# soedinglab/metaeuk

Hardware: AMD Instinct MI355X
Metric: prefilter+align ORF-fragments/sec (hits UNVERIFIED in this run: no CPU reference digest) (higher is better)
Workload: dtype packed i16 / i32 DP on u8 residues, i8 scores

## Files before the change

metaeuk_amd/csrc/mk_sw.hip:

```cpp
#include "mk_kernels.hpp"
#include <algorithm>
#include <mutex>

namespace mk {

template <int G>
__device__ __forceinline__ uint32_t shift_up(uint32_t top, uint32_t x, int laneInGroup) {
    if constexpr (G == 16) {
        return (uint32_t) __builtin_amdgcn_update_dpp((int) top, (int) x, 0x111 , 0xf, 0xf, false);
    } else if constexpr (G == 64) {
        return (uint32_t) __builtin_amdgcn_update_dpp((int) top, (int) x, 0x138 , 0xf, 0xf, false);
    } else {
        const uint32_t v = (uint32_t) __builtin_amdgcn_update_dpp((int) top, (int) x, 0x138 , 0xf, 0xf, false);
        return laneInGroup == 0 ? top : v;
    }
}

template <int G>
__device__ __forceinline__ uint32_t shift_up_zero(uint32_t x, int laneInGroup) {
    if constexpr (G == 16) return (uint32_t) __builtin_amdgcn_update_dpp((int) x, (int) x, 0x111 , 0xf, 0xf, true);
    else return shift_up<G>(0u, x, laneInGroup);
}

__device__ __forceinline__ int max3i(int a, int b, int c) { return max(max(a, b), c); }

template <int R>
__device__ __forceinline__ void load_scores(const int8_t *p, int (&sc)[R]) {
    if constexpr (R == 2) {
        const uint32_t w = *reinterpret_cast<const uint16_t *>(p);
        sc[0] = (int) (int8_t) (w & 0xFF);
        sc[1] = (int) (int8_t) (w >> 8);
    } else {
        const uint32_t *pw = reinterpret_cast<const uint32_t *>(p);
#pragma unroll
        for (int k = 0; k < R / 4; k++) {
            const uint32_t w = pw[k];
            sc[4 * k + 0] = (int) (int8_t) (w & 0xFF);
            sc[4 * k + 1] = (int) (int8_t) ((w >> 8) & 0xFF);
            sc[4 * k + 2] = (int) (int8_t) ((w >> 16) & 0xFF);
            sc[4 * k + 3] = (int) (int8_t) (w >> 24);
        }
    }
}

template <int G, int R, int BLOCK, bool SHARED>
__device__ __forceinline__ void sw_unit(const SwLaunch &L, const uint32_t unit, int8_t *smem, const int8_t *sMat) {
    constexpr int GPB = BLOCK / G;
    constexpr int ROWS = G * R;
    static_assert(!SHARED || BLOCK == 64, "shared-query mode runs one wave per workgroup");
    const int lane = threadIdx.x % G;
    const int grp = threadIdx.x / G;
    uint64_t jobId;
    bool have;
    SwJob job;
    uint32_t profQStart = 0; int profQStep = 1;
    if constexpr (SHARED) {
        const uint32_t w0 = L.wave_start[unit], w1 = L.wave_start[unit + 1];
        const uint32_t count = min((uint32_t) GPB, w1 - w0);
        have = (uint32_t) grp < count;
        jobId = (uint64_t) w0 + (have ? grp : 0);
        job = L.jobs[L.order ? (uint64_t) L.order[jobId] : jobId];
        if (!have) job.t_len = 0;
    } else {
        jobId = (uint64_t) unit * GPB + grp;
        have = jobId < L.n_jobs;
        if (have) job = L.jobs[L.order ? (uint64_t) L.order[jobId] : jobId];
        else { job.t_start = 0; job.q_start = 0; job.q_len = 0; job.t_len = 0; job.q_step = 1; job.t_step = 1; job.slot = 0; }
    }
    profQStart = job.q_start; profQStep = job.q_step;
    int8_t *prof = SHARED ? smem : smem + (size_t) grp * 24 * ROWS;
    const int go = L.gap_open, ge = L.gap_extend;
    const int qLen = (int) job.q_len, tLen = (int) job.t_len;
    const int nTiles = (qLen + ROWS - 1) / ROWS;
    uint32_t *border = L.boundary ? L.boundary + (jobId - L.boundary_job0) * (uint64_t) L.boundary_stride : nullptr;

    constexpr int NEED = (G - 1 + 15) / 16;
    int known = -1, after = 0;
    if constexpr (!SHARED) { if (L.known_score && have && nTiles == 1) known = L.known_score[job.slot]; }
    uint32_t bestKey = 0;
    int bestRow = 0;
    for (int tile = 0; tile < nTiles; tile++) {
        const int row0 = tile * ROWS;
        if (L.q_prof) {
            for (int i = SHARED ? (int) threadIdx.x : lane; i < ROWS * 6; i += SHARED ? BLOCK : G) {
                const int row = i / 6, w = i - row * 6;
                const int q = row0 + row;
                uint32_t v = 0;
                if (q < qLen) v = *reinterpret_cast<const uint32_t *>(L.q_prof + ((int64_t) profQStart + (int64_t) q * profQStep) * 32 + w * 4);
#pragma unroll
                for (int k = 0; k < 4; k++) if (4 * w + k < 22) prof[(4 * w + k) * ROWS + row] = (int8_t) (v >> (8 * k));
            }
        } else {
            uint8_t *sQ = reinterpret_cast<uint8_t *>(prof) + 22 * ROWS;
            int8_t *sB = reinterpret_cast<int8_t *>(sQ) + ROWS;
            for (int row = SHARED ? (int) threadIdx.x : lane; row < ROWS; row += SHARED ? BLOCK : G) {
                const int q = row0 + row;
                const bool real = q < qLen;
                const int64_t qi = (int64_t) profQStart + (int64_t) (real ? q : 0) * profQStep;
                sQ[row] = real ? L.q_res[qi] : (uint8_t) 255;
                sB[row] = real ? L.q_bias8[qi] : (int8_t) 0;
            }
            __builtin_amdgcn_fence(__ATOMIC_ACQ_REL, "wavefront");
            __builtin_amdgcn_wave_barrier();
            for (int idx = SHARED ? (int) threadIdx.x : lane; idx < 22 * ROWS; idx += SHARED ? BLOCK : G) {
                const int t = idx / ROWS, row = idx - t * ROWS;
                const uint32_t qc = sQ[row];
                prof[idx] = (t < 21 && qc != 255u) ? (int8_t) ((int) sMat[t * 21 + (int) qc] + (int) sB[row]) : (int8_t) 0;
            }
        }
        __builtin_amdgcn_fence(__ATOMIC_ACQ_REL, "wavefront");
        __builtin_amdgcn_wave_barrier();

        int H[R], E[R];
        uint32_t key[R];
#pragma unroll
        for (int r = 0; r < R; r++) { H[r] = 0; E[r] = 0; key[r] = 0; }
        uint32_t out0 = 0, out1 = 21u;
        int hupPrev = 0;
        const int steps = tLen > 0 ? tLen + G - 1 : 0;
        const bool readTop = (tile > 0);
        const bool writeBottom = (tile + 1 < nTiles);
        const int laneRow = (int) (threadIdx.x & 15u);
        const int64_t tBase = (int64_t) job.t_start;
        const int64_t tStep = (int64_t) job.t_step;
        const int tLast = max(tLen - 1, 0);
        uint32_t tq0 = L.t_res[tBase + (int64_t) min(laneRow, tLast) * tStep], tq1 = L.t_res[tBase + (int64_t) min(16 + laneRow, tLast) * tStep],
                 tq2 = L.t_res[tBase + (int64_t) min(32 + laneRow, tLast) * tStep];
        for (int s0 = 0; s0 < steps; s0 += 16) {
            uint32_t tcur = tq0;
            tq0 = tq1; tq1 = tq2;
            tq2 = L.t_res[tBase + (int64_t) min(s0 + 48 + laneRow, tLast) * tStep];
            const int sEnd = min(s0 + 16, steps);
            for (int s = s0; s < sEnd; s++) {
                uint32_t top0 = 0;
                const uint32_t top1 = s < tLen ? tcur : 21u;
                tcur = (uint32_t) __builtin_amdgcn_update_dpp(0, (int) tcur, 0x12F , 0xf, 0xf, false);
                if (readTop && lane == 0 && s < tLen) top0 = border[s];
                const uint32_t in0 = shift_up<G>(top0, out0, lane);
                const uint32_t tres = shift_up<G>(top1, out1, lane);
                const int hup = (int) (in0 & 0xFFFFu);
                int F = (int) (in0 >> 16);
                const int c = s - lane;
                const uint32_t cinv = 0x1FFFFu - (uint32_t) max(c, 0);
                int sc[R];
                load_scores<R>(prof + tres * ROWS + lane * R, sc);
                int dsave = hupPrev;
#pragma unroll
                for (int r = 0; r < R; r++) {
                    const int d = min(dsave + sc[r], 32767);
                    dsave = H[r];
                    const int h = max3i(d, E[r], F);
                    key[r] = max(key[r], ((uint32_t) h << 17) | cinv);
                    const int ho = h - go;
                    E[r] = max3i(E[r] - ge, ho, 0);
                    F = max3i(F - ge, ho, 0);
                    H[r] = h;
                }
                hupPrev = hup;
                out0 = (uint32_t) H[R - 1] | ((uint32_t) F << 16);
                out1 = tres;
                if (writeBottom && lane == G - 1 && c >= 0 && c < tLen) border[c] = out0;
            }
            if constexpr (!SHARED) {
                if (known > 0) {
                    bool seen = false;
#pragma unroll
                    for (int r = 0; r < R; r++) seen |= (key[r] >> 17) == (uint32_t) known;
                    const unsigned long long m = __ballot(seen);
                    const unsigned long long mine = G == 64 ? ~0ull : ((1ull << (G & 63)) - 1ull) << (((unsigned) threadIdx.x & 63u) / G * G);
                    if ((m & mine) != 0ull && ++after > NEED) break;
                }
            }
        }
#pragma unroll
        for (int r = 0; r < R; r++) {
            if (key[r] > bestKey) { bestKey = key[r]; bestRow = row0 + lane * R + r; }
        }
        __builtin_amdgcn_fence(__ATOMIC_ACQ_REL, "wavefront");
        __builtin_amdgcn_wave_barrier();
    }
#pragma unroll
    for (int m = G / 2; m >= 1; m >>= 1) {
        const uint32_t ok = (uint32_t) __shfl_xor((int) bestKey, m, G);
        const int orow = __shfl_xor(bestRow, m, G);
        if (ok > bestKey || (ok == bestKey && orow < bestRow)) { bestKey = ok; bestRow = orow; }
    }
    if (have && lane == 0) {
        SwOut o;
        o.score = (int32_t) (bestKey >> 17);
        o.end_col = o.score > 0 ? (int32_t) (0x1FFFFu - (bestKey & 0x1FFFFu)) : -1;
        o.end_row = o.score > 0 ? bestRow : -1;
        o.pad = 0;
        L.out[job.slot] = o;
    }
}

#ifndef MK_HELPER_PRIO
#define MK_HELPER_PRIO 3
#endif
template <int G, int R, int BLOCK, bool SHARED>
__global__ __launch_bounds__(BLOCK) void sw_kernel(SwLaunch L) {
    if (!SHARED && MK_HELPER_PRIO) __builtin_amdgcn_s_setprio(MK_HELPER_PRIO);
    extern __shared__ __attribute__((aligned(16))) int8_t smem[];
    __shared__ int8_t sMat[448];
    for (int k = (int) threadIdx.x; k < 441; k += BLOCK) sMat[k] = L.mat[k];
    __syncthreads();
    if constexpr (SHARED) {
        for (uint32_t done = 0; L.units_per_block == 0 || done < L.units_per_block; done++) {
            uint32_t u = 0;
            if (threadIdx.x == 0) u = atomicAdd(L.work_counter, 1u);
            u = (uint32_t) __builtin_amdgcn_readfirstlane((int) u);
            if ((uint64_t) u >= L.n_waves) break;
            sw_unit<G, R, BLOCK, true>(L, u, smem, sMat);
            __builtin_amdgcn_fence(__ATOMIC_ACQ_REL, "wavefront");
            __builtin_amdgcn_wave_barrier();
        }
    } else {
        sw_unit<G, R, BLOCK, false>(L, blockIdx.x, smem, sMat);
    }
}

template <int CLS>
__global__ __launch_bounds__(64) void sw_multi_kernel(SwLaunch L, const uint32_t *bounds, uint32_t *counter, int prio) {
    if (prio) __builtin_amdgcn_s_setprio(MK_HELPER_PRIO);
    extern __shared__ __attribute__((aligned(16))) int8_t smem[];
    __shared__ int8_t sMat[448];
    for (int k = (int) threadIdx.x; k < 441; k += 64) sMat[k] = L.mat[k];
    __builtin_amdgcn_fence(__ATOMIC_ACQ_REL, "wavefront");
    __builtin_amdgcn_wave_barrier();
    constexpr int C0 = CLS == 0 ? 0 : (CLS == 1 ? 3 : 7), C1 = CLS == 0 ? 3 : (CLS == 1 ? 7 : SW_NCFG), NC = C1 - C0;
    uint32_t lo[NC], nj[NC], ub[NC + 1];
    ub[0] = 0;
#pragma unroll
    for (int k = 0; k < NC; k++) {
        const int c = C1 - 1 - k;
        lo[k] = bounds[c]; nj[k] = bounds[c + 1] - lo[k];
        const uint32_t gpb = c >= 9 ? 1u : (c >= 7 ? 2u : 4u);
        ub[k + 1] = ub[k] + (nj[k] + gpb - 1u) / gpb;
    }
    for (;;) {
        uint32_t u = 0;
        if (threadIdx.x == 0) u = atomicAdd(counter, 1u);
        u = (uint32_t) __builtin_amdgcn_readfirstlane((int) u);
        if (u >= ub[NC]) break;
        int k = 0;
#pragma unroll
        for (int j = 1; j < NC; j++) if (u >= ub[j]) k = j;
        SwLaunch Lc = L;
        uint32_t first = 0, base = 0, count = 0;
#pragma unroll
        for (int j = 0; j < NC; j++) if (j == k) { first = lo[j]; base = ub[j]; count = nj[j]; }
        Lc.order = L.order + first; Lc.n_jobs = count;
        const uint32_t unit = u - base;
        const int c = C1 - 1 - k;
        if constexpr (CLS == 0) {
            if (c == 0) sw_unit<16, 2, 64, false>(Lc, unit, smem, sMat);
            else sw_unit<16, 4, 64, false>(Lc, unit, smem, sMat);
        } else if constexpr (CLS == 1) {
            if (c <= 4) sw_unit<16, 8, 64, false>(Lc, unit, smem, sMat);
            else sw_unit<16, 16, 64, false>(Lc, unit, smem, sMat);
        } else {
            if (c == 7) sw_unit<32, 12, 64, false>(Lc, unit, smem, sMat);
            else if (c == 8) sw_unit<32, 16, 64, false>(Lc, unit, smem, sMat);
            else if (c == 9) sw_unit<64, 12, 64, false>(Lc, unit, smem, sMat);
            else sw_unit<64, 16, 64, false>(Lc, unit, smem, sMat);
        }
        __builtin_amdgcn_fence(__ATOMIC_ACQ_REL, "wavefront");
        __builtin_amdgcn_wave_barrier();
    }
}

hipError_t launch_sw_multi(const SwLaunch &L, const uint32_t *bounds, uint32_t *counter, int cls, uint32_t blocks, hipStream_t stream, bool prio) {
    if (!L.order || !bounds || !counter || L.boundary || blocks == 0) return hipErrorInvalidValue;
    switch (cls) {
        case 0: hipLaunchKernelGGL((sw_multi_kernel<0>), dim3(blocks), dim3(64), (size_t) 64 * 24 * 4, stream, L, bounds, counter, prio ? 1 : 0); break;
        case 1: hipLaunchKernelGGL((sw_multi_kernel<1>), dim3(blocks), dim3(64), (size_t) 64 * 24 * 16, stream, L, bounds, counter, prio ? 1 : 0); break;
        case 2: hipLaunchKernelGGL((sw_multi_kernel<2>), dim3(blocks), dim3(64), (size_t) 64 * 24 * 16, stream, L, bounds, counter, prio ? 1 : 0); break;
        default: return hipErrorInvalidValue;
    }
    return hipGetLastError();
}

typedef short pk16 __attribute__((ext_vector_type(2)));
__device__ __forceinline__ pk16 pk_from(uint32_t v) { return __builtin_bit_cast(pk16, v); }
__device__ __forceinline__ uint32_t pk_bits(pk16 v) { return __builtin_bit_cast(uint32_t, v); }
__device__ __forceinline__ pk16 pk_max(pk16 a, pk16 b) { return __builtin_elementwise_max(a, b); }
__device__ __forceinline__ pk16 pk_splat(int v) { pk16 r; r.x = (short) v; r.y = (short) v; return r; }
typedef unsigned short pku16 __attribute__((ext_vector_type(2)));
__device__ __forceinline__ pk16 pk_subs0(pk16 a, pk16 b) {
    return __builtin_bit_cast(pk16, __builtin_elementwise_sub_sat(__builtin_bit_cast(pku16, a), __builtin_bit_cast(pku16, b)));
}

constexpr uint32_t SWT_MAX_ROWS = 256;
constexpr int SWT_MARGIN = 16, SWT_TAIL = 32, SWT_COL = 24;
__host__ __device__ inline size_t swt_image_bytes(int qLen) { return (size_t) (SWT_MARGIN + qLen + SWT_TAIL) * SWT_COL; }

template <int R>
__device__ __forceinline__ void swt_unit(const SwLaunch &L, const uint32_t w0, const uint32_t count, const int qLen) {
    constexpr int G = 16;
    constexpr int UNR = R <= 2 ? 16 : (R <= 4 ? 8 : (R <= 8 ? 4 : 2));
    extern __shared__ __attribute__((aligned(16))) int8_t smem[];
    const int lane = threadIdx.x % G, grp = threadIdx.x / G;
    const pk16 go2 = pk_splat(L.gap_open), ge2 = pk_splat(L.gap_extend), zero2 = pk_splat(0);
    const bool haveA = (uint32_t) (2 * grp) < count, haveB = (uint32_t) (2 * grp + 1) < count;
    const SwJob jobA = L.jobs[L.order[(uint64_t) w0 + (haveA ? 2 * grp : 0)]];
    const SwJob jobB = L.jobs[L.order[(uint64_t) w0 + (haveB ? 2 * grp + 1 : 0)]];
    const int tLenA = haveA ? (int) jobA.t_len : 0, tLenB = haveB ? (int) jobB.t_len : 0;
    uint32_t offA[R], offB[R];
#pragma unroll
    for (int r = 0; r < R; r++) {
        const int i = lane * R + r;
        const uint32_t a = i < tLenA ? (uint32_t) L.t_res[(int64_t) jobA.t_start + (int64_t) i * jobA.t_step] : 21u;
        const uint32_t b = i < tLenB ? (uint32_t) L.t_res[(int64_t) jobB.t_start + (int64_t) i * jobB.t_step] : 21u;
        offA[r] = min(a, 21u) + (uint32_t) ((SWT_MARGIN - lane) * SWT_COL); offB[r] = min(b, 21u) + (uint32_t) ((SWT_MARGIN - lane) * SWT_COL);
    }
    pk16 H[R], E[R], best[R];
#pragma unroll
    for (int r = 0; r < R; r++) { H[r] = zero2; E[r] = zero2; best[r] = zero2; }
    pk16 hupPrev = zero2;
    uint32_t outH = 0, outF = 0;
    const int steps = (qLen + G - 1 + 15) & ~15;
#pragma unroll 1
    for (int s0 = 0; s0 < steps; s0 += UNR) {
#pragma unroll
        for (int k = 0; k < UNR; k++) {
            const pk16 hup = pk_from(shift_up_zero<G>(outH, lane));
            pk16 F = pk_from(shift_up_zero<G>(outF, lane));
            pk16 dsave = hupPrev;
#pragma unroll
            for (int r = 0; r < R; r++) {
                const int sa = (int) smem[offA[r] + (uint32_t) (k * SWT_COL)], sb = (int) smem[offB[r] + (uint32_t) (k * SWT_COL)];
                const pk16 sc = pk_from(__builtin_amdgcn_perm((uint32_t) sb, (uint32_t) sa, 0x05040100u));
                const pk16 d = dsave + sc;
                dsave = H[r];
                const pk16 h = pk_max(pk_max(d, E[r]), F);
                best[r] = pk_max(best[r], h);
                const pk16 ho = pk_subs0(h, go2);
                E[r] = pk_max(pk_subs0(E[r], ge2), ho);
                F = pk_max(pk_subs0(F, ge2), ho);
                H[r] = h;
            }
            hupPrev = hup;
            outH = pk_bits(H[R - 1]);
            outF = pk_bits(F);
        }
#pragma unroll
        for (int r = 0; r < R; r++) { offA[r] += (uint32_t) (UNR * SWT_COL); offB[r] += (uint32_t) (UNR * SWT_COL); }
    }
    pk16 bAll = zero2;
#pragma unroll
    for (int r = 0; r < R; r++) bAll = pk_max(bAll, best[r]);
    uint32_t b = pk_bits(bAll);
#pragma unroll
    for (int m = G / 2; m >= 1; m >>= 1) b = pk_bits(pk_max(pk_from(b), pk_from((uint32_t) __shfl_xor((int) b, m, G))));
    uint32_t cA = 0x7FFFFFFFu, cB = 0x7FFFFFFFu;
#pragma unroll
    for (int r = R - 1; r >= 0; r--) {
        if ((pk_bits(best[r]) & 0xFFFFu) == (b & 0xFFFFu)) cA = (uint32_t) (lane * R + r);
        if ((pk_bits(best[r]) >> 16) == (b >> 16)) cB = (uint32_t) (lane * R + r);
    }
// ... 146 lines not shown
                for (int s = 0; s < 8; s++) {
                    if (run) {
                        const int k = __ffs((int) run) - 1;
                        run &= run - 1u;
                        jobIdx[s] = (uint32_t) __shfl((int) myJob, k, 64);
                        n++;
                    } else jobIdx[s] = jobIdx[0];
                }
                if constexpr (CLS == 0) {
                    if (tl <= 32u) swtp_unit<2>(L, jobIdx, n, (int) qLen);
                    else if (tl <= 48u) swtp_unit<3>(L, jobIdx, n, (int) qLen);
                    else swtp_unit<4>(L, jobIdx, n, (int) qLen);
                } else if constexpr (CLS == 1) {
                    if (tl <= 96u) swtp_unit<6>(L, jobIdx, n, (int) qLen);
                    else swtp_unit<8>(L, jobIdx, n, (int) qLen);
                } else {
                    if (tl <= 192u) swtp_unit<12>(L, jobIdx, n, (int) qLen);
                    else swtp_unit<16>(L, jobIdx, n, (int) qLen);
                }
            }
            __builtin_amdgcn_fence(__ATOMIC_ACQ_REL, "wavefront");
            __builtin_amdgcn_wave_barrier();
        }
    }
}

__device__ __forceinline__ uint32_t swt_longest(const SwLaunch &L, const uint32_t w0, const uint32_t count) {
    uint32_t tl = 0;
    if (threadIdx.x < count) tl = L.jobs[L.order[(uint64_t) w0 + threadIdx.x]].t_len;
#pragma unroll
    for (int m = 32; m >= 1; m >>= 1) tl = max(tl, (uint32_t) __shfl_xor((int) tl, m, 64));
    return tl;
}

template <int CLS>
__device__ __forceinline__ void swt_wave(const SwLaunch &L, const uint32_t w0, const uint32_t count, const uint32_t tl, int8_t *smem) {
    const SwJob j0 = L.jobs[L.order[w0]];
    const int qLen = (int) j0.q_len;
    swt_image(L, j0.q_start, j0.q_step, qLen, smem);
    if constexpr (CLS == 0) {
        if (tl <= 32u) swt_unit<2>(L, w0, count, qLen);
        else if (tl <= 48u) swt_unit<3>(L, w0, count, qLen);
        else swt_unit<4>(L, w0, count, qLen);
    } else if constexpr (CLS == 1) {
        if (tl <= 96u) swt_unit<6>(L, w0, count, qLen);
        else swt_unit<8>(L, w0, count, qLen);
    } else {
        if (tl <= 192u) swt_unit<12>(L, w0, count, qLen);
        else swt_unit<16>(L, w0, count, qLen);
    }
    __builtin_amdgcn_fence(__ATOMIC_ACQ_REL, "wavefront");
    __builtin_amdgcn_wave_barrier();
}

template <int CLS>
__global__ __launch_bounds__(64) void swt_kernel(SwLaunch L) {
    extern __shared__ __attribute__((aligned(16))) int8_t smem[];
    constexpr uint32_t LO = CLS == 0 ? 0u : (CLS == 1 ? 64u : 128u), HI = CLS == 0 ? 64u : (CLS == 1 ? 128u : SWT_MAX_ROWS);
    for (uint32_t done = 0; L.units_per_block == 0 || done < L.units_per_block; done++) {
        uint32_t u = 0;
        if (threadIdx.x == 0) u = atomicAdd(L.work_counter_t + 16 * CLS, 1u);
        u = (uint32_t) __builtin_amdgcn_readfirstlane((int) u);
        if ((uint64_t) u >= L.n_waves) break;
        const uint32_t w0 = L.wave_start[u], count = min(8u, L.wave_start[u + 1] - w0);
        const uint32_t tl = swt_longest(L, w0, count);
        if (tl > HI || (CLS > 0 && tl <= LO) || tl > L.t_max_rows) continue;
        swt_wave<CLS>(L, w0, count, tl, smem);
    }
}

template <int R, int RP = R, int G = 16>
__global__ __launch_bounds__(64) void swp_kernel(SwLaunch L) {
    constexpr int GPB = 64 / G, ROWS = G * RP;
    constexpr bool SAT = G * R * 127 > 32767;
    static_assert(RP >= R && RP % 2 == 0, "profile slots per lane: even and at least R");
    static_assert(G == 16 || G == 32, "a pair of DPs runs on one or two DPP rows");
    extern __shared__ __attribute__((aligned(16))) int8_t smem[];
    int16_t *prof = reinterpret_cast<int16_t *>(smem);
    int8_t *sMat = smem + (size_t) 22 * ROWS * sizeof(int16_t);
    uint8_t *sQ = reinterpret_cast<uint8_t *>(sMat + 448);
    int8_t *sB = reinterpret_cast<int8_t *>(sQ + ROWS);
    for (int k = (int) threadIdx.x; k < 441; k += 64) sMat[k] = L.mat[k];
    const int lane = threadIdx.x % G, grp = threadIdx.x / G;
    const pk16 go2 = pk_splat(L.gap_open), ge2 = pk_splat(L.gap_extend), zero2 = pk_splat(0);
    for (uint32_t done = 0; L.units_per_block == 0 || done < L.units_per_block; done++) {
        uint32_t u = 0;
        if (threadIdx.x == 0) u = atomicAdd(L.work_counter, 1u);
        u = (uint32_t) __builtin_amdgcn_readfirstlane((int) u);
        if ((uint64_t) u >= L.n_waves) break;
        const uint32_t wFirst = L.wave_start[u], wEnd = L.wave_start[u + 1];
        if (L.t_max_rows && swt_longest(L, wFirst, min(8u, wEnd - wFirst)) <= L.t_max_rows) continue;
        for (uint32_t w0 = wFirst; w0 < wEnd; w0 += (uint32_t) (2 * GPB)) {
        const uint32_t w1 = wEnd;
        const uint32_t count = min((uint32_t) (2 * GPB), w1 - w0);
        const bool haveA = (uint32_t) (2 * grp) < count, haveB = (uint32_t) (2 * grp + 1) < count;
        const SwJob jobA = L.jobs[L.order[(uint64_t) w0 + (haveA ? 2 * grp : 0)]];
        const SwJob jobB = L.jobs[L.order[(uint64_t) w0 + (haveB ? 2 * grp + 1 : 0)]];
        const int qLen = (int) jobA.q_len;
        const int tLenA = haveA ? (int) jobA.t_len : 0, tLenB = haveB ? (int) jobB.t_len : 0;
        if (L.q_prof) {
            for (int i = (int) threadIdx.x; i < ROWS * 6; i += 64) {
                const int slot = i / 6, w = i - slot * 6;
                const int row = RP == R ? slot : (slot / RP) * R + slot % RP;
                const bool real = row < qLen && (RP == R || slot % RP < R);
                uint32_t v = 0;
                if (real) v = *reinterpret_cast<const uint32_t *>(L.q_prof + ((int64_t) jobA.q_start + (int64_t) row * jobA.q_step) * 32 + w * 4);
#pragma unroll
                for (int k = 0; k < 4; k++) if (4 * w + k < 22) prof[(4 * w + k) * ROWS + slot] = (int16_t) (int8_t) (v >> (8 * k));
            }
        } else {
        for (int slot = (int) threadIdx.x; slot < ROWS; slot += 64) {
            const int row = RP == R ? slot : (slot / RP) * R + slot % RP;
            const bool real = row < qLen && (RP == R || slot % RP < R);
            const int64_t qi = (int64_t) jobA.q_start + (int64_t) (real ? row : 0) * jobA.q_step;
            sQ[slot] = real ? L.q_res[qi] : (uint8_t) 255;
            sB[slot] = real ? L.q_bias8[qi] : (int8_t) 0;
        }
        __builtin_amdgcn_fence(__ATOMIC_ACQ_REL, "wavefront");
        __builtin_amdgcn_wave_barrier();
        for (int idx = (int) threadIdx.x; idx < 22 * ROWS; idx += 64) {
            const int t = idx / ROWS, slot = idx - t * ROWS;
            const uint32_t qc = sQ[slot];
            prof[idx] = (t < 21 && qc != 255u) ? (int16_t) ((int) sMat[t * 21 + (int) qc] + (int) sB[slot]) : (int16_t) 0;
        }
        }
        __builtin_amdgcn_fence(__ATOMIC_ACQ_REL, "wavefront");
        __builtin_amdgcn_wave_barrier();

        pk16 H[R], E[R];
#pragma unroll
        for (int r = 0; r < R; r++) { H[r] = zero2; E[r] = zero2; }
        pk16 best = zero2, hupPrev = zero2;
        int roseA = 0, roseB = 0;
        constexpr uint32_t ROWB = (uint32_t) ROWS * 2u, NOCOL = 21u * ROWB | (21u * ROWB) << 16;
        uint32_t outH = 0, outF = 0, outRes = NOCOL;
        const int tMax = max(tLenA, tLenB);
        const int steps = tMax > 0 ? (tMax + G - 1 + 15) & ~15 : 0;
        const int laneRow = lane & 15;
        const int lastA = max(tLenA - 1, 0), lastB = max(tLenB - 1, 0);
        const int64_t baseA = (int64_t) jobA.t_start, baseB = (int64_t) jobB.t_start, stepA = jobA.t_step, stepB = jobB.t_step;
        const auto fetch = [&](int col) -> uint32_t {
            const uint32_t ra = col < tLenA ? (uint32_t) L.t_res[baseA + (int64_t) min(col, lastA) * stepA] : 21u;
            const uint32_t rb = col < tLenB ? (uint32_t) L.t_res[baseB + (int64_t) min(col, lastB) * stepB] : 21u;
            return ra * ROWB | (rb * ROWB) << 16;
        };
        const char *profLane = reinterpret_cast<const char *>(prof + lane * RP);
        uint32_t tq0 = fetch(laneRow), tq1 = fetch(16 + laneRow), tq2 = fetch(32 + laneRow);
        for (int s0 = 0; s0 < steps; s0 += 16) {
            uint32_t tcur = tq0;
            tq0 = tq1; tq1 = tq2;
            tq2 = fetch(s0 + 48 + laneRow);
            const uint32_t bestIn = pk_bits(best);
#pragma unroll
            for (int k = 0; k < 16; k++) {
                const uint32_t top = tcur;
                tcur = (uint32_t) __builtin_amdgcn_update_dpp(0, (int) tcur, 0x12F , 0xf, 0xf, false);
                const pk16 hup = pk_from(shift_up_zero<G>(outH, lane));
                pk16 F = pk_from(shift_up_zero<G>(outF, lane));
                const uint32_t tres = shift_up<G>(top, outRes, lane);
                const int16_t *pa = reinterpret_cast<const int16_t *>(profLane + (tres & 0xFFFFu)), *pb = reinterpret_cast<const int16_t *>(profLane + (tres >> 16));
                uint32_t wa[RP / 2], wb[RP / 2];
                if constexpr (RP % 4 == 0) {
                    const uint64_t *qa = reinterpret_cast<const uint64_t *>(__builtin_assume_aligned(pa, 8)), *qb = reinterpret_cast<const uint64_t *>(__builtin_assume_aligned(pb, 8));
#pragma unroll
                    for (int k = 0; k < RP / 4; k++) {
                        const uint64_t xa = qa[k], xb = qb[k];
                        wa[2 * k] = (uint32_t) xa; wa[2 * k + 1] = (uint32_t) (xa >> 32); wb[2 * k] = (uint32_t) xb; wb[2 * k + 1] = (uint32_t) (xb >> 32);
                    }
                } else {
#pragma unroll
                for (int k = 0; k < RP / 2; k++) { wa[k] = reinterpret_cast<const uint32_t *>(pa)[k]; wb[k] = reinterpret_cast<const uint32_t *>(pb)[k]; }
                }
                pk16 dsave = hupPrev;
#pragma unroll
                for (int r = 0; r < R; r++) {
                    const pk16 sc = pk_from(__builtin_amdgcn_perm(wb[r / 2], wa[r / 2], (r & 1) ? 0x07060302u : 0x05040100u));
                    const pk16 d = SAT ? __builtin_elementwise_add_sat(dsave, sc) : dsave + sc;
                    dsave = H[r];
                    const pk16 h = pk_max(pk_max(d, E[r]), F);
                    best = pk_max(best, h);
                    const pk16 ho = pk_subs0(h, go2);
                    E[r] = pk_max(pk_subs0(E[r], ge2), ho);
                    F = pk_max(pk_subs0(F, ge2), ho);
                    H[r] = h;
                }
                hupPrev = hup;
                outH = pk_bits(H[R - 1]);
                outF = pk_bits(F);
                outRes = tres;
            }
            const uint32_t rose = pk_bits(best) ^ bestIn;
            if (rose & 0xFFFFu) roseA = s0;
            if (rose >> 16) roseB = s0;
        }
        uint32_t b = pk_bits(best);
#pragma unroll
        for (int m = G / 2; m >= 1; m >>= 1) b = pk_bits(pk_max(pk_from(b), pk_from((uint32_t) __shfl_xor((int) b, m, G))));
        uint32_t cA = (pk_bits(best) & 0xFFFFu) == (b & 0xFFFFu) ? (uint32_t) max(roseA + 15 - lane, 0) : 0x7FFFFFFFu;
        uint32_t cB = (pk_bits(best) >> 16) == (b >> 16) ? (uint32_t) max(roseB + 15 - lane, 0) : 0x7FFFFFFFu;
#pragma unroll
        for (int m = G / 2; m >= 1; m >>= 1) {
            cA = min(cA, (uint32_t) __shfl_xor((int) cA, m, G));
            cB = min(cB, (uint32_t) __shfl_xor((int) cB, m, G));
        }
        if (lane == 0) {
            SwOut o;
            o.end_row = -1; o.pad = 0;
            if (haveA) { o.score = (int32_t) (int16_t) (b & 0xFFFFu); o.end_col = (int32_t) min(cA, (uint32_t) lastA); L.out[jobA.slot] = o; }
            if (haveB) { o.score = (int32_t) (int16_t) (b >> 16); o.end_col = (int32_t) min(cB, (uint32_t) lastB); L.out[jobB.slot] = o; }
        }
        __builtin_amdgcn_fence(__ATOMIC_ACQ_REL, "wavefront");
        __builtin_amdgcn_wave_barrier();
        }
    }
}

template <int R, int RP>
__global__ __launch_bounds__(64) void swq_kernel(SwLaunch L) {
    constexpr int G = 16, ROWS = G * RP, NDP = 8;
    static_assert(RP >= R && RP % 2 == 0 && G * R * 127 <= 32767, "small tiles only");
    extern __shared__ __attribute__((aligned(16))) int8_t smem[];
    int16_t *prof = reinterpret_cast<int16_t *>(smem);
    constexpr int PROF1 = 22 * ROWS;
    int8_t *sMat = smem + (size_t) NDP * PROF1 * sizeof(int16_t);
    uint8_t *sQ = reinterpret_cast<uint8_t *>(sMat + 448);
    int8_t *sB = reinterpret_cast<int8_t *>(sQ + NDP * ROWS);
    for (int k = (int) threadIdx.x; k < 441; k += 64) sMat[k] = L.mat[k];
    const int lane = threadIdx.x % G, grp = threadIdx.x / G;
    const pk16 go2 = pk_splat(L.gap_open), ge2 = pk_splat(L.gap_extend), zero2 = pk_splat(0);
    const uint64_t nUnits = (L.n_jobs + NDP - 1) / NDP;
    for (;;) {
        uint32_t u = 0;
        if (threadIdx.x == 0) u = atomicAdd(L.work_counter, 1u);
        u = (uint32_t) __builtin_amdgcn_readfirstlane((int) u);
        if ((uint64_t) u >= nUnits) break;
        const uint64_t j0 = (uint64_t) u * NDP;
        const uint64_t ja = j0 + 2 * grp, jb = ja + 1;
        const bool haveA = ja < L.n_jobs, haveB = jb < L.n_jobs;
        const SwJob jobA = L.jobs[L.order[haveA ? ja : j0]], jobB = L.jobs[L.order[haveB ? jb : j0]];
        const int tLenA = haveA ? (int) jobA.t_len : 0, tLenB = haveB ? (int) jobB.t_len : 0;
        const uint32_t SA = haveA ? (uint32_t) L.known_score[jobA.slot] & 0xFFFFu : 0xFFFFu, SB = haveB ? (uint32_t) L.known_score[jobB.slot] & 0xFFFFu : 0xFFFFu;
        const uint32_t S2 = SA | (SB << 16);
        for (int i = (int) threadIdx.x; i < NDP * ROWS; i += 64) {
            const int dp = i / ROWS, slot = i - dp * ROWS;
            const uint64_t j = j0 + (uint64_t) dp;
            uint8_t qc = 255; int8_t bc = 0;
            if (j < L.n_jobs) {
                const SwJob jj = L.jobs[L.order[j]];
                const int row = RP == R ? slot : (slot / RP) * R + slot % RP;
                if (row < (int) jj.q_len && (RP == R || slot % RP < R)) {
                    const int64_t qi = (int64_t) jj.q_start + (int64_t) row * jj.q_step;
                    qc = L.q_res[qi]; bc = L.q_bias8[qi];
                }
            }
            sQ[i] = qc; sB[i] = bc;
        }
        __builtin_amdgcn_fence(__ATOMIC_ACQ_REL, "wavefront");
        __builtin_amdgcn_wave_barrier();
        for (int i = (int) threadIdx.x; i < NDP * PROF1; i += 64) {
            const int dp = i / PROF1, rem = i - dp * PROF1, t = rem / ROWS, slot = rem - t * ROWS;
            const uint32_t qc = sQ[dp * ROWS + slot];
            prof[i] = (t < 21 && qc != 255u) ? (int16_t) ((int) sMat[t * 21 + (int) qc] + (int) sB[dp * ROWS + slot]) : (int16_t) 0;
        }
        __builtin_amdgcn_fence(__ATOMIC_ACQ_REL, "wavefront");
        __builtin_amdgcn_wave_barrier();

        pk16 H[R], E[R];
#pragma unroll
        for (int r = 0; r < R; r++) { H[r] = zero2; E[r] = zero2; }
        pk16 best = zero2, hupPrev = zero2;
        constexpr uint32_t ROWB = (uint32_t) ROWS * 2u, NOCOL = 21u * ROWB | (21u * ROWB) << 16;
        uint32_t outH = 0, outF = 0, outRes = NOCOL;
        const int tMax = max(tLenA, tLenB);
        const int steps = tMax > 0 ? (tMax + G - 1 + 15) & ~15 : 0;
        const int laneRow = lane & 15;
        const int lastA = max(tLenA - 1, 0), lastB = max(tLenB - 1, 0);
        const int64_t baseA = (int64_t) jobA.t_start, baseB = (int64_t) jobB.t_start, stepA = jobA.t_step, stepB = jobB.t_step;
        const auto fetch = [&](int col) -> uint32_t {
            const uint32_t ra = col < tLenA ? (uint32_t) L.t_res[baseA + (int64_t) min(col, lastA) * stepA] : 21u;
            const uint32_t rb = col < tLenB ? (uint32_t) L.t_res[baseB + (int64_t) min(col, lastB) * stepB] : 21u;
            return ra * ROWB | (rb * ROWB) << 16;
        };
        const char *profA = reinterpret_cast<const char *>(prof + (size_t) (2 * grp) * PROF1 + lane * RP);
        const char *profB = reinterpret_cast<const char *>(prof + (size_t) (2 * grp + 1) * PROF1 + lane * RP);
        uint32_t foundA = 0xFFFFFFFFu, foundB = 0xFFFFFFFFu;
        uint32_t closed2 = 0u;
        uint32_t tq0 = fetch(laneRow), tq1 = fetch(16 + laneRow), tq2 = fetch(32 + laneRow);
        for (int s0 = 0; s0 < steps; s0 += 16) {
            uint32_t tcur = tq0;
            tq0 = tq1; tq1 = tq2;
            tq2 = fetch(s0 + 48 + laneRow);
#pragma unroll
            for (int k = 0; k < 16; k++) {
                const uint32_t top = tcur;
                tcur = (uint32_t) __builtin_amdgcn_update_dpp(0, (int) tcur, 0x12F , 0xf, 0xf, false);
                const pk16 hup = pk_from(shift_up_zero<G>(outH, lane));
                pk16 F = pk_from(shift_up_zero<G>(outF, lane));
                const uint32_t tres = shift_up<G>(top, outRes, lane);
                const int16_t *pa = reinterpret_cast<const int16_t *>(profA + (tres & 0xFFFFu)), *pb = reinterpret_cast<const int16_t *>(profB + (tres >> 16));
                uint32_t wa[RP / 2], wb[RP / 2];
#pragma unroll
                for (int kk = 0; kk < RP / 2; kk++) { wa[kk] = reinterpret_cast<const uint32_t *>(pa)[kk]; wb[kk] = reinterpret_cast<const uint32_t *>(pb)[kk]; }
                pk16 dsave = hupPrev;
#pragma unroll
                for (int r = 0; r < R; r++) {
                    const pk16 sc = pk_from(__builtin_amdgcn_perm(wb[r / 2], wa[r / 2], (r & 1) ? 0x07060302u : 0x05040100u));
                    const pk16 d = dsave + sc;
                    dsave = H[r];
                    const pk16 h = pk_max(pk_max(d, E[r]), F);
                    best = pk_max(best, h);
                    const pk16 ho = pk_subs0(h, go2);
                    E[r] = pk_max(pk_subs0(E[r], ge2), ho);
                    F = pk_max(pk_subs0(F, ge2), ho);
                    H[r] = h;
                }
                hupPrev = hup;
                outH = pk_bits(H[R - 1]);
                outF = pk_bits(F);
                outRes = tres;
                const uint32_t x = (pk_bits(best) ^ S2) | closed2;
                const uint32_t hit = (x - 0x00010001u) & ~x & 0x80008000u;
                if (__builtin_amdgcn_ballot_w64(hit != 0u) != 0ull) {
                    const int c = s0 + k - lane;
                    if ((x & 0xFFFFu) == 0u) {
                        int row = 0;
#pragma unroll
                        for (int r = R - 1; r >= 0; r--) if ((pk_bits(H[r]) & 0xFFFFu) == SA) row = r;
                        foundA = ((uint32_t) c << 12) | (uint32_t) (lane * R + row);
                        closed2 |= 0x1u;
                    }
                    if ((x >> 16) == 0u) {
                        int row = 0;
#pragma unroll
                        for (int r = R - 1; r >= 0; r--) if ((pk_bits(H[r]) >> 16) == SB) row = r;
                        foundB = ((uint32_t) c << 12) | (uint32_t) (lane * R + row);
                        closed2 |= 0x10000u;
                    }
                }
            }
        }
#pragma unroll
        for (int m = G / 2; m >= 1; m >>= 1) {
            foundA = min(foundA, (uint32_t) __shfl_xor((int) foundA, m, G));
            foundB = min(foundB, (uint32_t) __shfl_xor((int) foundB, m, G));
        }
        if (lane == 0) {
            SwOut o;
            o.pad = 0;
            if (haveA) { const bool ok = foundA != 0xFFFFFFFFu; o.score = ok ? (int32_t) SA : 0; o.end_col = ok ? (int32_t) (foundA >> 12) : -1; o.end_row = ok ? (int32_t) (foundA & 0xFFFu) : -1; L.out[jobA.slot] = o; }
            if (haveB) { const bool ok = foundB != 0xFFFFFFFFu; o.score = ok ? (int32_t) SB : 0; o.end_col = ok ? (int32_t) (foundB >> 12) : -1; o.end_row = ok ? (int32_t) (foundB & 0xFFFu) : -1; L.out[jobB.slot] = o; }
        }
        __builtin_amdgcn_fence(__ATOMIC_ACQ_REL, "wavefront");
        __builtin_amdgcn_wave_barrier();
    }
}

hipError_t launch_sw_known(const SwLaunch &L, int cfg, hipStream_t stream) {
    if (!L.order || !L.work_counter || !L.known_score || cfg < 0 || cfg >= SW_NCFG || !sw_cfg_known(cfg)) return hipErrorInvalidValue;
    if (L.n_jobs == 0) return hipSuccess;
    const uint64_t nUnits = (L.n_jobs + 7) / 8;
    const uint64_t grid = std::min<uint64_t>(nUnits, L.persistent_blocks ? L.persistent_blocks : nUnits);
    const int rows = sw_cfg_rows(cfg);
    const size_t prows = rows == 48 ? 64 : rows;
    const size_t lds = (size_t) 8 * 22 * prows * sizeof(int16_t) + 448 + 2 * 8 * prows;
    switch (rows) {
        case 32: hipLaunchKernelGGL((swq_kernel<2, 2>), dim3((unsigned) grid), dim3(64), lds, stream, L); break;
        case 48: hipLaunchKernelGGL((swq_kernel<3, 4>), dim3((unsigned) grid), dim3(64), lds, stream, L); break;
        case 64: hipLaunchKernelGGL((swq_kernel<4, 4>), dim3((unsigned) grid), dim3(64), lds, stream, L); break;
        default: return hipErrorInvalidValue;
    }
    return hipGetLastError();
}

hipError_t launch_sw_score(const SwLaunch &L, int cfg, hipStream_t stream) {
    if (!L.wave_start || !L.work_counter || !L.order || cfg < 0 || cfg >= SW_NCFG || !sw_cfg_packed(cfg)) return hipErrorInvalidValue;
    if (L.n_waves == 0) return hipSuccess;
    const uint64_t grid = L.units_per_block ? (L.n_waves + L.units_per_block - 1) / L.units_per_block
                                            : std::min<uint64_t>(L.n_waves, L.persistent_blocks ? L.persistent_blocks : L.n_waves);
    const int rows = sw_cfg_rows(cfg);
    const size_t prows = rows == 48 ? 64 : rows;
    const size_t lds = (size_t) 22 * prows * sizeof(int16_t) + 448 + 2 * prows;
    if (L.t_max_rows) {
        if (!L.work_counter_t || !L.q_prof || !L.narrow || L.t_max_rows > SWT_MAX_ROWS) return hipErrorInvalidValue;
        hipLaunchKernelGGL(swt_kernel<0>, dim3((unsigned) grid), dim3(64), swt_image_bytes(rows), stream, L);
        if (L.t_max_rows > 64u) hipLaunchKernelGGL(swt_kernel<1>, dim3((unsigned) grid), dim3(64), swt_image_bytes(rows), stream, L);
        if (L.t_max_rows > 128u) hipLaunchKernelGGL(swt_kernel<2>, dim3((unsigned) grid), dim3(64), swt_image_bytes(rows), stream, L);
    }
    switch (rows) {
        case 32: hipLaunchKernelGGL((swp_kernel<2>), dim3((unsigned) grid), dim3(64), lds, stream, L); break;
        case 48: hipLaunchKernelGGL((swp_kernel<3, 4>), dim3((unsigned) grid), dim3(64), lds, stream, L); break;
        case 64: hipLaunchKernelGGL((swp_kernel<4>), dim3((unsigned) grid), dim3(64), lds, stream, L); break;
        case 96: hipLaunchKernelGGL((swp_kernel<6>), dim3((unsigned) grid), dim3(64), lds, stream, L); break;
        case 128: hipLaunchKernelGGL((swp_kernel<8>), dim3((unsigned) grid), dim3(64), lds, stream, L); break;
        case 192: hipLaunchKernelGGL((swp_kernel<12>), dim3((unsigned) grid), dim3(64), lds, stream, L); break;
        case 256: hipLaunchKernelGGL((swp_kernel<16>), dim3((unsigned) grid), dim3(64), lds, stream, L); break;
        case 384: if (L.narrow) hipLaunchKernelGGL((swp_kernel<24, 24, 16>), dim3((unsigned) grid), dim3(64), lds, stream, L);
                  else hipLaunchKernelGGL((swp_kernel<12, 12, 32>), dim3((unsigned) grid), dim3(64), lds, stream, L);
                  break;
        case 512: hipLaunchKernelGGL((swp_kernel<16, 16, 32>), dim3((unsigned) grid), dim3(64), lds, stream, L); break;
        case 768: hipLaunchKernelGGL((swp_kernel<24, 24, 32>), dim3((unsigned) grid), dim3(64), lds, stream, L); break;
        default: return hipErrorInvalidValue;
    }
    return hipGetLastError();
}

hipError_t launch_sw_tpos(const SwLaunch &L, int rows, uint32_t blocksPerClass, hipStream_t stream) {
    if (!L.q_prof || !L.order || !L.known_score || rows <= 0) return hipErrorInvalidValue;
    if (L.n_jobs == 0) return hipSuccess;
    const unsigned grid = (unsigned) std::min<uint64_t>((L.n_jobs + 7) / 8, std::max<uint32_t>(1u, blocksPerClass));
    hipLaunchKernelGGL(swtp_kernel<0>, dim3(grid), dim3(64), swt_image_bytes(rows), stream, L);
    hipLaunchKernelGGL(swtp_kernel<1>, dim3(grid), dim3(64), swt_image_bytes(rows), stream, L);
    hipLaunchKernelGGL(swtp_kernel<2>, dim3(grid), dim3(64), swt_image_bytes(rows), stream, L);
    return hipGetLastError();
}

template <int G, int R, int BLOCK>
static hipError_t launch_one(const SwLaunch &L, hipStream_t stream) {
    if (L.wave_start) {
        const size_t lds = (size_t) 24 * G * R;
        if (L.n_waves == 0) return hipSuccess;
        const uint64_t grid = L.units_per_block ? (L.n_waves + L.units_per_block - 1) / L.units_per_block
                                                : std::min<uint64_t>(L.n_waves, L.persistent_blocks ? L.persistent_blocks : L.n_waves);
        hipLaunchKernelGGL((sw_kernel<G, R, 64, true>), dim3((unsigned) grid), dim3(64), lds, stream, L);
        return hipGetLastError();
    }
    constexpr int GPB = BLOCK / G;
    const size_t lds = (size_t) GPB * 24 * G * R;
    const uint64_t blocks = (L.n_jobs + GPB - 1) / GPB;
    if (blocks == 0) return hipSuccess;
    if (lds > 48 * 1024) {
        static std::once_flag once;
        static hipError_t attrErr = hipSuccess;
        std::call_once(once, [&] { attrErr = hipFuncSetAttribute(reinterpret_cast<const void *>(&sw_kernel<G, R, BLOCK, false>), hipFuncAttributeMaxDynamicSharedMemorySize, (int) lds); });
        if (attrErr != hipSuccess) return attrErr;
    }
    hipLaunchKernelGGL((sw_kernel<G, R, BLOCK, false>), dim3((unsigned) blocks), dim3(BLOCK), lds, stream, L);
    return hipGetLastError();
}

hipError_t launch_sw(const SwLaunch &L, int cfg, hipStream_t stream) {
    if (cfg < 0 || cfg >= SW_NCFG) return hipErrorInvalidValue;
    switch (sw_cfg_rows(cfg)) {
#ifndef MK_SW_POS_BLOCK_S
#define MK_SW_POS_BLOCK_S 256
#define MK_SW_POS_BLOCK_L 128
#endif
        case 32: return launch_one<16, 2, MK_SW_POS_BLOCK_S>(L, stream);
        case 48:
        case 64: return launch_one<16, 4, MK_SW_POS_BLOCK_S>(L, stream);
        case 96:
        case 128: return launch_one<16, 8, MK_SW_POS_BLOCK_S>(L, stream);
        case 192:
        case 256: return launch_one<16, 16, MK_SW_POS_BLOCK_L>(L, stream);
        case 384: return launch_one<32, 12, MK_SW_POS_BLOCK_L>(L, stream);
        case 512: return launch_one<32, 16, MK_SW_POS_BLOCK_L>(L, stream);
        case 768: return launch_one<64, 12, MK_SW_POS_BLOCK_L>(L, stream);
        case 1024: return launch_one<64, 16, MK_SW_POS_BLOCK_L>(L, stream);
        default: return hipErrorInvalidValue;
    }
}

__global__ __launch_bounds__(256) void ungapped_kernel(UngappedLaunch L) {
    __shared__ int8_t smat[21 * 21 + 3];
    for (int i = threadIdx.x; i < 21 * 21; i += blockDim.x) smat[i] = L.mat[i];
    __syncthreads();
    const uint64_t id = (uint64_t) blockIdx.x * blockDim.x + threadIdx.x;
    if (id >= L.n_jobs) return;
    const UngappedJob j = L.jobs[id];
    const int best = ungapped_score(smat, L.q_res + j.q_start, L.q_corr + j.q_start, j.q_len, L.t_masked + j.t_start, j.t_len, j.diagonal & 0xFFFFu);
    L.out[id] = best;
}

hipError_t launch_ungapped(const UngappedLaunch &L, hipStream_t stream) {
    if (L.n_jobs == 0) return hipSuccess;
    const uint64_t blocks = (L.n_jobs + 255) / 256;
    hipLaunchKernelGGL(ungapped_kernel, dim3((unsigned) blocks), dim3(256), 0, stream, L);
    return hipGetLastError();
}

}
```

Measured before the change: 2.533 million.

## Stage target residue columns in an LDS ring instead of DPP shift chains

Target residues are now written 16 columns at a time into a small per-wave LDS ring buffer. Each lane then reads its own diagonal column index directly, which replaces the per-step DPP row shift of the residue and the separate carry of the residue down the anti-diagonal. The aim is to cut the cross-lane shift instructions and the extra register traffic from the inner DP loop. In exchange it adds an LDS read per step, a wave barrier per 16-step block, and extra LDS allocation in every launch path.

Measured after the change: 2.546 million (median of 6 runs). About the same (+0.5%).

```diff
diff --git a/metaeuk_amd/csrc/mk_sw.hip b/metaeuk_amd/csrc/mk_sw.hip
--- a/metaeuk_amd/csrc/mk_sw.hip
+++ b/metaeuk_amd/csrc/mk_sw.hip
@@ -22,16 +22,45 @@
     else return shift_up<G>(0u, x, laneInGroup);
 }
 
+typedef __attribute__((address_space(3))) const uint32_t lds_cu32;
+typedef __attribute__((address_space(3))) const uint16_t lds_cu16;
+typedef __attribute__((address_space(3))) const int8_t lds_ci8;
+template <typename T>
+__device__ __forceinline__ T *lds_opaque(T *p) {
+    uint32_t a = (uint32_t) (uintptr_t) p;
+    asm volatile("" : "+v"(a));
+    return (T *) (uintptr_t) a;
+}
+
+constexpr int COL_RING = 64, COL_RING_WORDS = COL_RING + 16;
+template <int RING = COL_RING, typename T>
+__device__ __forceinline__ void col_ring_put(T *ring, const int col0, const int laneRow, const T v) {
+    const int w = col0 & (RING - 1);
+    ring[w + laneRow] = v;
+    if (w == 0) ring[RING + laneRow] = v;
+}
+template <int RING = COL_RING, typename T>
+__device__ __forceinline__ auto col_ring_at(const T *ring, const int col) {
+    typedef __attribute__((address_space(3))) const T lds_ct;
+    return lds_opaque((lds_ct *) (ring + (col & (RING - 1))));
+}
+constexpr size_t sw_ring_bytes(int G, int block) { return (size_t) (block / G) * ((G == 64 ? 2 * COL_RING : COL_RING) + 16); }
+template <int G, int RING = COL_RING, typename T>
+__device__ __forceinline__ void col_ring_reset(T *ring, const int lane, const T nocol) {
+    constexpr int N = (G + 15) & ~15;
+    for (int i = lane; i < N; i += G) ring[RING - N + i] = nocol;
+}
+
 __device__ __forceinline__ int max3i(int a, int b, int c) { return max(max(a, b), c); }
 
-template <int R>
-__device__ __forceinline__ void load_scores(const int8_t *p, int (&sc)[R]) {
+template <int R, typename P>
+__device__ __forceinline__ void load_scores(P p, int (&sc)[R]) {
     if constexpr (R == 2) {
-        const uint32_t w = *reinterpret_cast<const uint16_t *>(p);
+        const uint32_t w = *(lds_cu16 *) p;
         sc[0] = (int) (int8_t) (w & 0xFF);
         sc[1] = (int) (int8_t) (w >> 8);
     } else {
-        const uint32_t *pw = reinterpret_cast<const uint32_t *>(p);
+        lds_cu32 *pw = (lds_cu32 *) p;
 #pragma unroll
         for (int k = 0; k < R / 4; k++) {
             const uint32_t w = pw[k];
@@ -69,6 +98,9 @@
     }
     profQStart = job.q_start; profQStep = job.q_step;
     int8_t *prof = SHARED ? smem : smem + (size_t) grp * 24 * ROWS;
+    constexpr int RING = G == 64 ? 2 * COL_RING : COL_RING;
+    constexpr uint8_t NOCOL = 21;
+    uint8_t *ring = reinterpret_cast<uint8_t *>(smem + (size_t) (SHARED ? 1 : GPB) * 24 * ROWS) + grp * (RING + 16);
     const int go = L.gap_open, ge = L.gap_extend;
     const int qLen = (int) job.q_len, tLen = (int) job.t_len;
     const int nTiles = (qLen + ROWS - 1) / ROWS;
@@ -115,7 +147,7 @@
         uint32_t key[R];
 #pragma unroll
         for (int r = 0; r < R; r++) { H[r] = 0; E[r] = 0; key[r] = 0; }
-        uint32_t out0 = 0, out1 = 21u;
+        uint32_t out0 = 0;
         int hupPrev = 0;
         const int steps = tLen > 0 ? tLen + G - 1 : 0;
         const bool readTop = (tile > 0);
@@ -124,26 +156,35 @@
         const int64_t tBase = (int64_t) job.t_start;
         const int64_t tStep = (int64_t) job.t_step;
         const int tLast = max(tLen - 1, 0);
-        uint32_t tq0 = L.t_res[tBase + (int64_t) min(laneRow, tLast) * tStep], tq1 = L.t_res[tBase + (int64_t) min(16 + laneRow, tLast) * tStep],
-                 tq2 = L.t_res[tBase + (int64_t) min(32 + laneRow, tLast) * tStep];
+        const auto fetch = [&](int col) -> uint8_t { return L.t_res[tBase + (int64_t) min(col, tLast) * tStep]; };
+        const auto entry = [&](uint8_t r, int col) -> uint8_t { return col < tLen ? r : NOCOL; };
+        lds_ci8 *profLane = lds_opaque((lds_ci8 *) (prof + lane * R));
+        col_ring_reset<G, RING>(ring, lane, NOCOL);
+        constexpr bool DEEP = R < 12;
+        const uint8_t t0 = fetch(laneRow);
+        uint8_t tq0 = fetch(16 + laneRow), tq1 = DEEP ? fetch(32 + laneRow) : NOCOL;
+        col_ring_put<RING>(ring, 0, laneRow, entry(t0, laneRow));
         for (int s0 = 0; s0 < steps; s0 += 16) {
-            uint32_t tcur = tq0;
-            tq0 = tq1; tq1 = tq2;
-            tq2 = L.t_res[tBase + (int64_t) min(s0 + 48 + laneRow, tLast) * tStep];
+            col_ring_put<RING>(ring, s0 + 16, laneRow, entry(tq0, s0 + 16 + laneRow));
+            if constexpr (DEEP) { tq0 = tq1; tq1 = fetch(s0 + 48 + laneRow); }
+            else tq0 = fetch(s0 + 32 + laneRow);
+            __builtin_amdgcn_fence(__ATOMIC_ACQ_REL, "wavefront");
+            __builtin_amdgcn_wave_barrier();
+            auto cols = col_ring_at<RING>(ring, s0 - lane);
+            uint32_t tnext = cols[0];
             const int sEnd = min(s0 + 16, steps);
             for (int s = s0; s < sEnd; s++) {
                 uint32_t top0 = 0;
-                const uint32_t top1 = s < tLen ? tcur : 21u;
-                tcur = (uint32_t) __builtin_amdgcn_update_dpp(0, (int) tcur, 0x12F , 0xf, 0xf, false);
+                const uint32_t tres = tnext;
+                tnext = *++cols;
                 if (readTop && lane == 0 && s < tLen) top0 = border[s];
                 const uint32_t in0 = shift_up<G>(top0, out0, lane);
-                const uint32_t tres = shift_up<G>(top1, out1, lane);
                 const int hup = (int) (in0 & 0xFFFFu);
                 int F = (int) (in0 >> 16);
                 const int c = s - lane;
                 const uint32_t cinv = 0x1FFFFu - (uint32_t) max(c, 0);
                 int sc[R];
-                load_scores<R>(prof + tres * ROWS + lane * R, sc);
+                load_scores<R>(profLane + tres * ROWS, sc);
                 int dsave = hupPrev;
 #pragma unroll
                 for (int r = 0; r < R; r++) {
@@ -158,7 +199,6 @@
                 }
                 hupPrev = hup;
                 out0 = (uint32_t) H[R - 1] | ((uint32_t) F << 16);
-                out1 = tres;
                 if (writeBottom && lane == G - 1 && c >= 0 && c < tLen) border[c] = out0;
             }
             if constexpr (!SHARED) {
@@ -272,10 +312,12 @@
 
 hipError_t launch_sw_multi(const SwLaunch &L, const uint32_t *bounds, uint32_t *counter, int cls, uint32_t blocks, hipStream_t stream, bool prio) {
     if (!L.order || !bounds || !counter || L.boundary || blocks == 0) return hipErrorInvalidValue;
+    constexpr size_t ringBytes = sw_ring_bytes(16, 64);
+    static_assert(sw_ring_bytes(32, 64) <= ringBytes && sw_ring_bytes(64, 64) <= ringBytes, "ring bytes of a wave");
     switch (cls) {
-        case 0: hipLaunchKernelGGL((sw_multi_kernel<0>), dim3(blocks), dim3(64), (size_t) 64 * 24 * 4, stream, L, bounds, counter, prio ? 1 : 0); break;
-        case 1: hipLaunchKernelGGL((sw_multi_kernel<1>), dim3(blocks), dim3(64), (size_t) 64 * 24 * 16, stream, L, bounds, counter, prio ? 1 : 0); break;
-        case 2: hipLaunchKernelGGL((sw_multi_kernel<2>), dim3(blocks), dim3(64), (size_t) 64 * 24 * 16, stream, L, bounds, counter, prio ? 1 : 0); break;
+        case 0: hipLaunchKernelGGL((sw_multi_kernel<0>), dim3(blocks), dim3(64), (size_t) 64 * 24 * 4 + ringBytes, stream, L, bounds, counter, prio ? 1 : 0); break;
+        case 1: hipLaunchKernelGGL((sw_multi_kernel<1>), dim3(blocks), dim3(64), (size_t) 64 * 24 * 16 + ringBytes, stream, L, bounds, counter, prio ? 1 : 0); break;
+        case 2: hipLaunchKernelGGL((sw_multi_kernel<2>), dim3(blocks), dim3(64), (size_t) 64 * 24 * 16 + ringBytes, stream, L, bounds, counter, prio ? 1 : 0); break;
         default: return hipErrorInvalidValue;
     }
     return hipGetLastError();
@@ -588,6 +630,7 @@
     int8_t *sB = reinterpret_cast<int8_t *>(sQ + ROWS);
     for (int k = (int) threadIdx.x; k < 441; k += 64) sMat[k] = L.mat[k];
     const int lane = threadIdx.x % G, grp = threadIdx.x / G;
+    uint32_t *ring = reinterpret_cast<uint32_t *>(sB + ROWS) + grp * COL_RING_WORDS;
     const pk16 go2 = pk_splat(L.gap_open), ge2 = pk_splat(L.gap_extend), zero2 = pk_splat(0);
     for (uint32_t done = 0; L.units_per_block == 0 || done < L.units_per_block; done++) {
         uint32_t u = 0;
@@ -639,7 +682,7 @@
         pk16 best = zero2, hupPrev = zero2;
         int roseA = 0, roseB = 0;
         constexpr uint32_t ROWB = (uint32_t) ROWS * 2u, NOCOL = 21u * ROWB | (21u * ROWB) << 16;
-        uint32_t outH = 0, outF = 0, outRes = NOCOL;
+        uint32_t outH = 0, outF = 0;
         const int tMax = max(tLenA, tLenB);
         const int steps = tMax > 0 ? (tMax + G - 1 + 15) & ~15 : 0;
         const int laneRow = lane & 15;
@@ -651,19 +694,22 @@
             return ra * ROWB | (rb * ROWB) << 16;
         };
         const char *profLane = reinterpret_cast<const char *>(prof + lane * RP);
-        uint32_t tq0 = fetch(laneRow), tq1 = fetch(16 + laneRow), tq2 = fetch(32 + laneRow);
-        for (int s0 = 0; s0 < steps; s0 += 16) {
-            uint32_t tcur = tq0;
+        col_ring_reset<G>(ring, lane, NOCOL);
+        uint32_t tq0 = NOCOL, tq1 = NOCOL, tq2 = NOCOL;
+        for (int s0 = -64; s0 < steps; s0 += 16) {
+            if (s0 >= -16) col_ring_put(ring, s0 + 16, laneRow, tq0);
             tq0 = tq1; tq1 = tq2;
-            tq2 = fetch(s0 + 48 + laneRow);
+            tq2 = fetch(s0 + 64 + laneRow);
+            if (s0 < 0) continue;
+            __builtin_amdgcn_fence(__ATOMIC_ACQ_REL, "wavefront");
+            __builtin_amdgcn_wave_barrier();
+            lds_cu32 *cols = col_ring_at(ring, s0 - lane);
             const uint32_t bestIn = pk_bits(best);
 #pragma unroll
             for (int k = 0; k < 16; k++) {
-                const uint32_t top = tcur;
-                tcur = (uint32_t) __builtin_amdgcn_update_dpp(0, (int) tcur, 0x12F , 0xf, 0xf, false);
                 const pk16 hup = pk_from(shift_up_zero<G>(outH, lane));
                 pk16 F = pk_from(shift_up_zero<G>(outF, lane));
-                const uint32_t tres = shift_up<G>(top, outRes, lane);
+                const uint32_t tres = cols[k];
                 const int16_t *pa = reinterpret_cast<const int16_t *>(profLane + (tres & 0xFFFFu)), *pb = reinterpret_cast<const int16_t *>(profLane + (tres >> 16));
                 uint32_t wa[RP / 2], wb[RP / 2];
                 if constexpr (RP % 4 == 0) {
@@ -693,7 +739,6 @@
                 hupPrev = hup;
                 outH = pk_bits(H[R - 1]);
                 outF = pk_bits(F);
-                outRes = tres;
             }
             const uint32_t rose = pk_bits(best) ^ bestIn;
             if (rose & 0xFFFFu) roseA = s0;
@@ -733,6 +778,7 @@
     int8_t *sB = reinterpret_cast<int8_t *>(sQ + NDP * ROWS);
     for (int k = (int) threadIdx.x; k < 441; k += 64) sMat[k] = L.mat[k];
     const int lane = threadIdx.x % G, grp = threadIdx.x / G;
+    uint32_t *ring = reinterpret_cast<uint32_t *>(sB + NDP * ROWS) + grp * COL_RING_WORDS;
     const pk16 go2 = pk_splat(L.gap_open), ge2 = pk_splat(L.gap_extend), zero2 = pk_splat(0);
     const uint64_t nUnits = (L.n_jobs + NDP - 1) / NDP;
     for (;;) {
@@ -776,7 +822,7 @@
         for (int r = 0; r < R; r++) { H[r] = zero2; E[r] = zero2; }
         pk16 best = zero2, hupPrev = zero2;
         constexpr uint32_t ROWB = (uint32_t) ROWS * 2u, NOCOL = 21u * ROWB | (21u * ROWB) << 16;
-        uint32_t outH = 0, outF = 0, outRes = NOCOL;
+        uint32_t outH = 0, outF = 0;
         const int tMax = max(tLenA, tLenB);
         const int steps = tMax > 0 ? (tMax + G - 1 + 15) & ~15 : 0;
         const int laneRow = lane & 15;
@@ -791,18 +837,21 @@
         const char *profB = reinterpret_cast<const char *>(prof + (size_t) (2 * grp + 1) * PROF1 + lane * RP);
         uint32_t foundA = 0xFFFFFFFFu, foundB = 0xFFFFFFFFu;
         uint32_t closed2 = 0u;
-        uint32_t tq0 = fetch(laneRow), tq1 = fetch(16 + laneRow), tq2 = fetch(32 + laneRow);
-        for (int s0 = 0; s0 < steps; s0 += 16) {
-            uint32_t tcur = tq0;
+        col_ring_reset<G>(ring, lane, NOCOL);
+        uint32_t tq0 = NOCOL, tq1 = NOCOL, tq2 = NOCOL;
+        for (int s0 = -64; s0 < steps; s0 += 16) {
+            if (s0 >= -16) col_ring_put(ring, s0 + 16, laneRow, tq0);
             tq0 = tq1; tq1 = tq2;
-            tq2 = fetch(s0 + 48 + laneRow);
+            tq2 = fetch(s0 + 64 + laneRow);
+            if (s0 < 0) continue;
+            __builtin_amdgcn_fence(__ATOMIC_ACQ_REL, "wavefront");
+            __builtin_amdgcn_wave_barrier();
+            lds_cu32 *cols = col_ring_at(ring, s0 - lane);
 #pragma unroll
             for (int k = 0; k < 16; k++) {
-                const uint32_t top = tcur;
-                tcur = (uint32_t) __builtin_amdgcn_update_dpp(0, (int) tcur, 0x12F , 0xf, 0xf, false);
                 const pk16 hup = pk_from(shift_up_zero<G>(outH, lane));
                 pk16 F = pk_from(shift_up_zero<G>(outF, lane));
-                const uint32_t tres = shift_up<G>(top, outRes, lane);
+                const uint32_t tres = cols[k];
                 const int16_t *pa = reinterpret_cast<const int16_t *>(profA + (tres & 0xFFFFu)), *pb = reinterpret_cast<const int16_t *>(profB + (tres >> 16));
                 uint32_t wa[RP / 2], wb[RP / 2];
 #pragma unroll
@@ -823,7 +872,6 @@
                 hupPrev = hup;
                 outH = pk_bits(H[R - 1]);
                 outF = pk_bits(F);
-                outRes = tres;
                 const uint32_t x = (pk_bits(best) ^ S2) | closed2;
                 const uint32_t hit = (x - 0x00010001u) & ~x & 0x80008000u;
                 if (__builtin_amdgcn_ballot_w64(hit != 0u) != 0ull) {
@@ -868,7 +916,7 @@
     const uint64_t grid = std::min<uint64_t>(nUnits, L.persistent_blocks ? L.persistent_blocks : nUnits);
     const int rows = sw_cfg_rows(cfg);
     const size_t prows = rows == 48 ? 64 : rows;
-    const size_t lds = (size_t) 8 * 22 * prows * sizeof(int16_t) + 448 + 2 * 8 * prows;
+    const size_t lds = (size_t) 8 * 22 * prows * sizeof(int16_t) + 448 + 2 * 8 * prows + 4 * COL_RING_WORDS * sizeof(uint32_t);
     switch (rows) {
         case 32: hipLaunchKernelGGL((swq_kernel<2, 2>), dim3((unsigned) grid), dim3(64), lds, stream, L); break;
         case 48: hipLaunchKernelGGL((swq_kernel<3, 4>), dim3((unsigned) grid), dim3(64), lds, stream, L); break;
@@ -885,7 +933,7 @@
                                             : std::min<uint64_t>(L.n_waves, L.persistent_blocks ? L.persistent_blocks : L.n_waves);
     const int rows = sw_cfg_rows(cfg);
     const size_t prows = rows == 48 ? 64 : rows;
-    const size_t lds = (size_t) 22 * prows * sizeof(int16_t) + 448 + 2 * prows;
+    const size_t lds = (size_t) 22 * prows * sizeof(int16_t) + 448 + 2 * prows + 4 * COL_RING_WORDS * sizeof(uint32_t);
     if (L.t_max_rows) {
         if (!L.work_counter_t || !L.q_prof || !L.narrow || L.t_max_rows > SWT_MAX_ROWS) return hipErrorInvalidValue;
         hipLaunchKernelGGL(swt_kernel<0>, dim3((unsigned) grid), dim3(64), swt_image_bytes(rows), stream, L);
@@ -923,7 +971,7 @@
 template <int G, int R, int BLOCK>
 static hipError_t launch_one(const SwLaunch &L, hipStream_t stream) {
     if (L.wave_start) {
-        const size_t lds = (size_t) 24 * G * R;
+        const size_t lds = (size_t) 24 * G * R + sw_ring_bytes(G, 64);
         if (L.n_waves == 0) return hipSuccess;
         const uint64_t grid = L.units_per_block ? (L.n_waves + L.units_per_block - 1) / L.units_per_block
                                                 : std::min<uint64_t>(L.n_waves, L.persistent_blocks ? L.persistent_blocks : L.n_waves);
@@ -931,7 +979,7 @@
         return hipGetLastError();
     }
     constexpr int GPB = BLOCK / G;
-    const size_t lds = (size_t) GPB * 24 * G * R;
+    const size_t lds = (size_t) GPB * 24 * G * R + sw_ring_bytes(G, BLOCK);
     const uint64_t blocks = (L.n_jobs + GPB - 1) / GPB;
     if (blocks == 0) return hipSuccess;
     if (lds > 48 * 1024) {
```
